# BartvLaatum/GreenLight-Gym2

Measured on AMD Instinct MI355X. Metric: TomatoEnv env-steps/sec, higher is better.
Workload: dtype f32

## Files before the change

### greenlight-gym2_amd/csrc/glgym.hip

```cpp
#include <hip/hip_runtime.h>

#include <cmath>
#include <cstdio>
#include <cstdlib>
#include <cstring>
#include <new>
#include <string>
#include <vector>

#include "glgym.h"
#include "gl_model.hpp"
#include "gl_model_quad.hpp"
#include "gl_reward.hpp"
#include "glgym_bdf.h"
#include "glgym_rng.h"
#include "glgym_plan.h"

using namespace glm;

namespace {

thread_local std::string g_err;

#define HIPCHK(expr)                                                                                   \
    do {                                                                                               \
        hipError_t e_ = (expr);                                                                        \
        if (e_ != hipSuccess) {                                                                        \
            g_err = std::string(#expr) + ": " + hipGetErrorString(e_);                                 \
            return GLGYM_EHIP;                                                                         \
        }                                                                                              \
    } while (0)

constexpr int WAVE = 64;

#include "gl_default_const.inc"
static_assert(sizeof(ModelConst<float>) == sizeof(kDefaultConstF32_image), "regenerate gl_default_const.inc");
static_assert(sizeof(ModelConst<double>) == sizeof(kDefaultConstF64_image), "regenerate gl_default_const.inc");
template <class T> struct DefaultConst;
template <> struct DefaultConst<float> {
    static constexpr ModelConst<float> value = __builtin_bit_cast(ModelConst<float>, kDefaultConstF32_bits);
};
template <> struct DefaultConst<double> {
    static constexpr ModelConst<double> value = __builtin_bit_cast(ModelConst<double>, kDefaultConstF64_bits);
};
__constant__ const ModelConst<float> g_default_f32 = __builtin_bit_cast(ModelConst<float>, kDefaultConstF32_bits);
__constant__ const ModelConst<double> g_default_f64 = __builtin_bit_cast(ModelConst<double>, kDefaultConstF64_bits);
template <class T> __device__ __forceinline__ const ModelConst<T>& device_default();
template <> __device__ __forceinline__ const ModelConst<float>& device_default<float>() { return g_default_f32; }
template <> __device__ __forceinline__ const ModelConst<double>& device_default<double>() { return g_default_f64; }

template <class T> struct RewardConst : RewardConstBase<T> {};

template <class T> struct StepArgsT {
    int B, ld;
    T* x; T* u;
// ... 482 lines not shown
    T k[NX];
    rhs<T, true, PIPE>(x0, s, m, cr, k);
    for (int i = 0; i < NX; ++i) dx[(size_t)b * NX + i] = (double)k[i];
}

template <class T, bool PER_ENV_CROP, bool PIPE = false, int SCH = 0>
__global__ __launch_bounds__(WAVE) void evalf_kernel(const double* x, const double* u, const double* d,
                                                     const double* crop, int B, T dt, int n_sub, T gasR, T tCanMin,
                                                     ModelConst<T> m, double* x_next, int rhs_only, int nd,
                                                     int* n_failed, int verify, int window)
{
    const int b = blockIdx.x * WAVE + threadIdx.x;
    if (b >= B) return;
    T x0[NX], uu[NU], dd[7];
    for (int i = 0; i < NX; ++i) x0[i] = T(x[(size_t)b * NX + i]);
    for (int i = 0; i < NU; ++i) uu[i] = T(u[(size_t)b * NU + i]);
    for (int i = 0; i < 7; ++i) dd[i] = T(d[(size_t)b * nd + i]);
    CropConst<T> crLocal;
    if (PER_ENV_CROP) {
        T pc[NCROP];
        for (int i = 0; i < NCROP; ++i) pc[i] = T(crop[(size_t)b * NCROP + i]);
        make_crop_const<T, T>(pc, gasR, tCanMin, crLocal);
    }
    const CropConst<T>& cr = PER_ENV_CROP ? crLocal : m.crop;
    StepCoef<T> s;
    precompute(uu, dd, m, cr, s);
    if (PIPE) {
        const T tPipe = T(d[(size_t)b * nd + 10]), swOff = T(d[(size_t)b * nd + 12]);
        s.pipeTrack = ((tPipe < T(1)) || (swOff > T(0))) ? T(0) : T(1);
        s.tPipeSet = tPipe;
    }
    if (rhs_only) {
        T k[NX];
        rhs<T, true, PIPE>(x0, s, m, cr, k);
        for (int i = 0; i < NX; ++i) x_next[(size_t)b * NX + i] = (double)k[i];
        return;
    }
    T del[NX];
    bool failed;
    rk4_delta_guarded<T, PIPE, gl_order(SCH), SchemeWin<T, SCH>::value>(x0, s, m, cr, dt, n_sub, del, &failed, nullptr, verify != 0, nullptr, window);
    for (int i = 0; i < NX; ++i)
        x_next[(size_t)b * NX + i] = failed ? __builtin_nan("") : (double)x0[i] + (double)del[i];
    if (failed) atomicAdd(n_failed, 1);
}

template <class T> struct ObsArgsT {
    int B, ld;
    const T* x; const T* u; const T* weather; int weather_rows;
    const int* w_off; const int* timestep; const float* start_day;
    int Np; float* obs; double doy_inc, hod_inc;
    const unsigned char* mask; float* term_obs;
    int nd;
    int moff[6], dim;
};

#ifndef GL_OBS_ROWS
#define GL_OBS_ROWS 16
#endif
constexpr int OBS_ROWS = GL_OBS_ROWS, OBS_NCORE = 23, OBS_MAX_NP = 128;
template <class T> __global__ __launch_bounds__(256) void obs_kernel(ObsArgsT<T> a)
{
    constexpr int ROWS = OBS_ROWS, NCORE = OBS_NCORE;
    extern __shared__ float4 span4[];
    float* span = reinterpret_cast<float*>(span4);
    const int tid = threadIdx.x;
    const int dim = a.dim;
    const float kPpm = (float)(8.3144598 / (101325.0 * 44.01e-3));
    for (int rb = blockIdx.x * ROWS; rb < a.B; rb += gridDim.x * ROWS) {
        const int nrows = min(ROWS, a.B - rb);
        if (a.mask) {
            int any = 0;
            for (int r = 0; r < nrows; ++r) any |= a.mask[rb + r];
            if (!any) continue;
        }
        int base_r[ROWS];
#pragma unroll
        for (int r = 0; r < ROWS; ++r) {
            const int b = rb + (r < nrows ? r : 0);
            const int ts = a.timestep[b];
            base_r[r] = a.w_off[b] + (ts > 0 ? ts - 1 : 0);
        }
        for (int e = tid; e < ROWS * NCORE; e += 256) {
            const int r = e / NCORE, j = e - r * NCORE;
            const int b = rb + (r < nrows ? r : 0);
            const int ts = a.timestep[b];
            const int k = ts > 0 ? ts - 1 : 0;
            int base = 0;
#pragma unroll
            for (int rr = 0; rr < ROWS; ++rr) base = (rr == r) ? base_r[rr] : base;
            base = base >= a.weather_rows ? a.weather_rows - 1 : (base < 0 ? 0 : base);
            const T* wrow = a.weather + (size_t)base * a.nd;
            const int xi = j == 0 ? 0 : j == 1 ? 2 : j == 2 ? 15 : j == 3 ? 9 : j == 4 ? 21 : j == 5 ? 25 : 26;
            const T* p1 = j < 7 ? a.x + (size_t)xi * a.ld + b
                                : (j < 13 ? a.u + (size_t)(j - 7) * a.ld + b : wrow + (j < 18 ? j - 13 : 0));
            const T* p2 = j < 13 ? a.x + (size_t)2 * a.ld + b : wrow + 1;
            const float prim = (float)*p1, aux = (float)*p2, sday = a.start_day[b];
            const float sat = 610.78f * __builtin_amdgcn_exp2f(1.44269504f * 17.2694f * aux * __builtin_amdgcn_rcpf(aux + 238.3f));
            const float rh = fminf(fmaxf(100.0f * prim * __builtin_amdgcn_rcpf(sat), 0.0f), 100.0f);
            const float ppm = kPpm * (aux + 273.15f) * prim;
            const int c = j - 18;
            const double rev = (c <= 2) ? ((double)sday + (double)ts * a.doy_inc) * (1.0 / 365.0)
                                        : (double)ts * a.hod_inc * (1.0 / 24.0);
            const float fr = (float)(rev - floor(rev));
            const float clk = (c == 1 || c == 3) ? __builtin_amdgcn_sinf(fr) : __builtin_amdgcn_cosf(fr);
            float v = prim;
            v = (j == 0 || j == 16) ? ppm : v;
            v = (j == 2 || j == 15) ? rh : v;
            v = (j == 18) ? (float)k : v;
            v = (j > 18) ? clk : v;
            const int mo = j < 4 ? a.moff[0] : j < 7 ? a.moff[1] : j < 13 ? a.moff[2] : j < 18 ? a.moff[3] : a.moff[4];
            const int jl = j < 4 ? j : j < 7 ? j - 4 : j < 13 ? j - 7 : j < 18 ? j - 13 : j - 18;
            if (r < nrows && mo >= 0) span[r * dim + mo + jl] = v;
        }
        const int nf = a.moff[5] >= 0 ? 5 * a.Np : 0;
        for (int q = tid; q < nf; q += 256) {
            const int i = q / 5, c = q - i * 5;
            float v[ROWS];
#pragma unroll
            for (int r = 0; r < ROWS; ++r) {
                int row = base_r[r] + 1 + i;
                row = row >= a.weather_rows ? a.weather_rows - 1 : (row < 0 ? 0 : row);
                v[r] = (float)a.weather[(size_t)row * a.nd + c];
            }
#pragma unroll
            for (int r = 0; r < ROWS; ++r)
                if (r < nrows) span[r * dim + a.moff[5] + q] = v[r];
        }
        __syncthreads();
        float* out = a.obs + (size_t)rb * dim;
        if (!a.mask && nrows == ROWS) {
            const int n4 = (ROWS * dim) >> 2;
            float4* out4 = reinterpret_cast<float4*>(out);
            typedef float v4f __attribute__((ext_vector_type(4)));
            const v4f* src4 = reinterpret_cast<const v4f*>(span4);
            v4f* dst4 = reinterpret_cast<v4f*>(out4);
            for (int e = tid; e < n4; e += 256) __builtin_nontemporal_store(src4[e], &dst4[e]);
        } else {
            for (int r = 0; r < nrows; ++r) {
                if (a.mask && !a.mask[rb + r]) continue;
                for (int jj = tid; jj < dim; jj += 256) {
                    const size_t e = (size_t)r * dim + jj;
                    if (a.mask && a.term_obs) a.term_obs[(size_t)rb * dim + e] = out[e];
                    out[e] = span[e];
                }
            }
        }
        __syncthreads();
    }
}

template <class T>
__global__ __launch_bounds__(256) void rule_based_kernel(glgym_rule_cfg c, int B, int ld, const T* __restrict__ x,
                                                         const T* __restrict__ weather, int weather_rows,
                                                         const int* __restrict__ w_off, const int* __restrict__ timestep,
                                                         const float* __restrict__ start_day, const double* hour,
                                                         const double* doy_in, double doy_inc, double hod_inc,
                                                         T* __restrict__ control, int nd)
{
    const int b = blockIdx.x * blockDim.x + threadIdx.x;
    if (b >= B) return;
    const int ts = timestep[b];
    int row = w_off[b] + ts;
    row = row >= weather_rows ? weather_rows - 1 : (row < 0 ? 0 : row);
    const T* w = weather + (size_t)row * nd;
    const double iGlob = (double)w[0], tOut = (double)w[1], dli = (double)w[7], isDay = (double)w[8],
                 isDaySmooth = (double)w[9];
    const double co2Air = (double)x[b], tAir = (double)x[(size_t)2 * ld + b], vpAir = (double)x[(size_t)15 * ld + b];
    const double hod = hour ? hour[b] : fmod((double)ts * hod_inc, 24.0);
    const double doy = doy_in ? doy_in[b] : (double)start_day[b] + (double)ts * doy_inc;
    auto pband = [](double v, double sp, double band, double lo, double hi) {
        return lo + (hi - lo) * (1.0 / (1.0 + exp(-2.0 / band * 4.605170185988092 * (v - sp - band * 0.5))));
    };
    const double tod = c.lamps_on <= c.lamps_off ? (double)(c.lamps_on < hod && hod < c.lamps_off)
                                                 : (double)(c.lamps_on < hod || hod < c.lamps_off);
    const double doy_ok = c.lamps_day_start <= c.lamps_day_stop
                              ? (double)(c.lamps_day_start < doy && doy < c.lamps_day_stop)
                              : (double)(c.lamps_day_start < doy || doy < c.lamps_day_stop);
    const double below_dli = (double)(dli < c.lamp_rad_sum_limit);
    const double lamp_no_cons = (double)(iGlob < c.lamps_off_sun) * below_dli * tod * doy_ok;
    const double sw_on = fmax(0.0, fmin(1.0, hod - c.lamps_on + 1.0));
    const double sw_off = fmax(0.0, fmin(1.0, c.lamps_off - hod + 1.0));
    const double both = c.lamps_on == c.lamps_off ? 0.0
                        : (c.lamps_on < c.lamps_off ? fmin(sw_on, sw_off) : fmax(sw_on, sw_off));
    const double smooth_lamp = both * below_dli * doy_ok;
    const double day_inside = fmax(smooth_lamp, isDay);
    const double heat_sp = day_inside * c.temp_setpoint_day + (1.0 - day_inside) * c.temp_setpoint_night +
                           c.heat_correction * lamp_no_cons;
    const double heat_max = heat_sp + c.heat_deadzone;
    const double co2_sp = day_inside * c.co2_day;
    const double co2_ppm = 1e6 * 8.3144598 * (tAir + 273.15) * (1e-6 * co2Air) / (101325.0 * 44.01e-3);
    const double rh_in = 100.0 * vpAir / (610.78 * exp(17.2694 * tAir / (tAir + 238.3)));
    const double vent_heat = pband(tAir, heat_max, c.vent_heat_Pband, 0, 1);
    const double vent_rh = pband(rh_in, c.rh_max + 0.0 * c.mech_dehumid_Pband, c.vent_rh_Pband, 0, 1);
    const double vent_cold = pband(tAir, heat_sp - c.t_vent_off, c.vent_cold_Pband, 1, 0);
    const double th_sp = isDay * c.thScrSpDay + (1.0 - isDay) * c.thScrSpNight;
    const double th_cold = pband(tOut, th_sp, c.thScrPband, 0, 1);
    const double th_heat = pband(tAir, heat_sp + c.thScrDeadZone, -c.thScrPband, 1, 0);
    const double th_rh = fmax(pband(rh_in, c.rhMax + c.thScrRh, c.thScrRhPband, 1, 0), 1.0 - vent_cold);
    const double lamp_on = lamp_no_cons * pband(tAir, heat_max + c.lampExtraHeat, -0.5, 0, 1) *
                           (isDaySmooth + (1.0 - isDaySmooth)) *
// ... 914 lines not shown
        g_err = "glgym_step: GLGYM_INTEGRATOR_BDF does not support GLGYM_ODE_PIPE";
        return GLGYM_EINVAL;
    }
    glbdf::BdfEnvArgs<T> k;
    k.ld = a->ld;
    k.x = (T*)a->x; k.u = (T*)a->u; k.action = a->action; k.control = (const T*)a->control;
    k.weather = (const T*)a->weather; k.weather_rows = a->weather_rows; k.nd = h->nd;
    k.w_off = a->w_off; k.timestep = a->timestep; k.crop_p = (const T*)a->crop_p; k.N = a->N;
    k.reward = (T*)a->reward; k.info = (T*)a->info; k.done = a->done; k.step_flags = a->step_flags;
    k.dt = h->dt; k.rtol = h->rtol; k.atol = h->atol; k.max_steps = h->max_steps;
    k.gasR = h->p[39]; k.tCanMin = h->p[162];
    k.du = h->du;
    for (int j = 0; j < NU; ++j) { k.u_min[j] = h->u_min[j]; k.u_max[j] = h->u_max[j]; }
    HIPCHK(bdf_env_launch<T>(k, a->B, h->md, rw, a->metrics, st));
    return GLGYM_OK;
}

extern "C" int glgym_step(glgym_handle h, const glgym_step_args* a, void* stream)
{
    if (!h || !a) { g_err = "glgym_step: null handle / arguments"; return GLGYM_EINVAL; }
    if (a->struct_size != (int32_t)sizeof(glgym_step_args)) {
        g_err = "glgym_step: glgym_step_args.struct_size is " + std::to_string(a->struct_size) + ", this library expects " +
                std::to_string(sizeof(glgym_step_args)) + " (ABI " + std::to_string(GLGYM_ABI_VERSION) + "): rebuild against include/glgym.h";
        return GLGYM_EINVAL;
    }
    if (a->B < 1 || a->ld < a->B || !a->x || !a->u || !a->weather || !a->w_off || !a->timestep ||
        !a->reward || !a->done || (!a->action) == (!a->control) || a->weather_rows < 1) {
        g_err = "glgym_step: bad arguments (exactly one of action/control, ld >= B, non-null state/outputs)";
        return GLGYM_EINVAL;
    }
    if (h->step_integrator == GLGYM_INTEGRATOR_BDF) {
        DeviceGuard dev_guard(h);
        return h->dtype == GLGYM_F32 ? launch_step_bdf<float>(h, a, h->rf, (hipStream_t)stream)
                                     : launch_step_bdf<double>(h, a, h->rd, (hipStream_t)stream);
    }
    if (h->integrator != GLGYM_INTEGRATOR_EXPLICIT) {
        g_err = "glgym_step: GLGYM_INTEGRATOR_BDF is available to glgym_evalF only; set GLGYM_INTEGRATOR_EXPLICIT for env-steps";
        return GLGYM_EINVAL;
    }
    DeviceGuard dev_guard(h);
    hipStream_t st = (hipStream_t)stream;
    return h->dtype == GLGYM_F32 ? launch_step<float>(h, a, h->mf, h->rf, st)
                                 : launch_step<double>(h, a, h->md, h->rd, st);
}

static const int OBS_MODULE_SIZE[6] = {4, 3, 6, 5, 5, 0};

template <class T> static int launch_obs(glgym_handle h, const glgym_obs_args* a, hipStream_t st)
{
    ObsArgsT<T> k;
    k.B = a->B; k.ld = a->ld; k.x = (const T*)a->x; k.u = (const T*)a->u; k.weather = (const T*)a->weather;
    k.weather_rows = a->weather_rows; k.w_off = a->w_off; k.timestep = a->timestep; k.start_day = a->start_day;
    k.Np = a->Np; k.obs = a->obs; k.mask = a->mask; k.term_obs = a->term_obs; k.doy_inc = std::fmod(h->dt / 86400.0, 365.0); k.hod_inc = h->dt / 3600.0; k.nd = h->nd;
    int blocks = (a->B + OBS_ROWS - 1) / OBS_ROWS;
    static const int cap = [] { const char* e = std::getenv("GLGYM_OBS_BLOCKS"); return e ? std::atoi(e) : 4096; }();
    if (blocks > cap) blocks = cap;
    for (int m = 0; m < 6; ++m) k.moff[m] = -1;
    k.dim = 0;
    for (int i = 0; i < h->n_obs_modules; ++i) {
        const int m = h->obs_modules[i];
        k.moff[m] = k.dim;
        k.dim += m == GLGYM_OBS_FORECAST ? 5 * a->Np : OBS_MODULE_SIZE[m];
    }
    const size_t lds = (size_t)OBS_ROWS * k.dim * sizeof(float);
    hipLaunchKernelGGL((obs_kernel<T>), dim3(blocks), dim3(256), lds, st, k);
    HIPCHK(hipGetLastError());
    return GLGYM_OK;
}



extern "C" int glgym_weather(glgym_handle h, const glgym_weather_args* a, void* stream)
{
    DeviceGuard dev_guard(h);
    if (!h || !a || a->n_raw < 3 || a->n_out < 1 || a->nd < ND || !a->time || !a->i_glob || !a->t_out || !a->rh || !a->wind ||
        !a->t_sky || !a->out || !a->workspace) {
        g_err = "glgym_weather: bad arguments (>= 3 raw samples, nd >= 10, non-null device pointers)";
        return GLGYM_EINVAL;
    }
    hipStream_t st = (hipStream_t)stream;
    const int n = a->n_raw;
    double* W = a->workspace;
    double* D = a->workspace + (size_t)10 * n;
    hipLaunchKernelGGL(weather_convert_kernel, dim3((n + 255) / 256), dim3(256), 0, st, n, a->time, a->i_glob, a->t_out,
                       a->rh, a->wind, a->t_sky, a->co2_ppm, W);
    hipLaunchKernelGGL(weather_scan_kernel, dim3(1), dim3(64), 0, st, n, a->time, W);
    hipLaunchKernelGGL(pchip_slopes_kernel, dim3((n + 255) / 256, 10), dim3(256), 0, st, n, 10, a->time, W, D);
    if (a->nd > ND) {
        HIPCHK(hipMemsetAsync(a->out, 0, (size_t)a->n_out * a->nd * (h->dtype == GLGYM_F32 ? 4 : 8), st));
    }
    const dim3 grid((a->n_out + 255) / 256, 10);
    if (h->dtype == GLGYM_F32)
        hipLaunchKernelGGL((pchip_eval_kernel<float>), grid, dim3(256), 0, st, n, 10, a->n_out, a->nd, a->time, W, D,
                           (float*)a->out);
    else
        hipLaunchKernelGGL((pchip_eval_kernel<double>), grid, dim3(256), 0, st, n, 10, a->n_out, a->nd, a->time, W, D,
                           (double*)a->out);
    HIPCHK(hipGetLastError());
    return GLGYM_OK;
}

extern "C" int glgym_vecnorm(glgym_handle h, const glgym_vecnorm_args* a, void* stream)
{
    DeviceGuard dev_guard(h);
    if (!h || !a || a->B < 1 || a->dim < 1 || !a->obs || !a->obs_out || !a->obs_mean || !a->obs_var || !a->obs_count ||
        !a->workspace || (a->reward && (!a->reward_out || !a->ret_stats || !a->returns))) {
        g_err = "glgym_vecnorm: bad arguments";
        return GLGYM_EINVAL;
    }
    hipStream_t st = (hipStream_t)stream;
    const int B = a->B, dim = a->dim;
    double* acc = a->workspace;
    double* acc2 = a->workspace + (size_t)VN_REP * 2 * dim;
    HIPCHK(hipMemsetAsync(a->workspace, 0, ((size_t)VN_REP * 2 * dim + 2) * sizeof(double), st));
    const int do_obs = a->training && a->norm_obs, do_ret = a->training && a->reward != nullptr;
    int col_threads = (dim + WAVE - 1) / WAVE * WAVE;
    if (col_threads > 1024) col_threads = 1024;
    if (do_obs) {
        int blocks = (B + 63) / 64;
        if (blocks > 1024) blocks = 1024;
        hipLaunchKernelGGL(vecnorm_moments_kernel, dim3(blocks), dim3(col_threads), 0, st, a->obs, B, dim, acc);
    }
    if (do_ret) {
        if (h->dtype == GLGYM_F32)
            hipLaunchKernelGGL((vecnorm_returns_kernel<float>), dim3((B + 255) / 256), dim3(256), 0, st,
                               (const float*)a->reward, a->returns, B, a->gamma, acc2);
        else
            hipLaunchKernelGGL((vecnorm_returns_kernel<double>), dim3((B + 255) / 256), dim3(256), 0, st,
                               (const double*)a->reward, a->returns, B, a->gamma, acc2);
    }
    double* scale = acc;
    if (do_obs || do_ret || a->norm_obs)
        hipLaunchKernelGGL(vecnorm_merge_kernel, dim3(1), dim3(1024), 0, st, a->obs_mean, a->obs_var, a->obs_count, acc, dim, B,
                           a->ret_stats, acc2, do_obs, do_ret, a->epsilon, a->norm_obs ? scale : nullptr);
    const size_t total = (size_t)B * dim;
    if (a->norm_obs) {
        int blocks = (B + 15) / 16;
        if (blocks > 8192) blocks = 8192;
        hipLaunchKernelGGL(vecnorm_apply_kernel, dim3(blocks), dim3(col_threads), 0, st, a->obs, a->obs_out, B, dim,
                           a->obs_mean, scale, a->clip_obs);
    } else if (a->obs_out != a->obs) {
        HIPCHK(hipMemcpyAsync(a->obs_out, a->obs, total * sizeof(float), hipMemcpyDeviceToDevice, st));
    }
    if (a->reward) {
        if (h->dtype == GLGYM_F32)
            hipLaunchKernelGGL((vecnorm_reward_kernel<float>), dim3((B + 255) / 256), dim3(256), 0, st,
                               (const float*)a->reward, a->reward_out, a->returns, a->done, B, a->ret_stats, a->epsilon,
                               a->clip_reward, a->norm_reward);
        else
            hipLaunchKernelGGL((vecnorm_reward_kernel<double>), dim3((B + 255) / 256), dim3(256), 0, st,
                               (const double*)a->reward, a->reward_out, a->returns, a->done, B, a->ret_stats, a->epsilon,
                               a->clip_reward, a->norm_reward);
    }
    HIPCHK(hipGetLastError());
    return GLGYM_OK;
}

extern "C" {

int glgym_obs(glgym_handle h, const glgym_obs_args* a, void* stream)
{
    DeviceGuard dev_guard(h);
    if (!h || !a || a->B < 1 || a->ld < a->B || !a->x || !a->u || !a->weather || !a->w_off || !a->timestep ||
        !a->start_day || !a->obs || a->Np < 0 || a->Np > OBS_MAX_NP) {
        g_err = "glgym_obs: bad arguments (null pointer, ld < B, or Np outside 0..128)";
        return GLGYM_EINVAL;
    }
    hipStream_t st = (hipStream_t)stream;
    return h->dtype == GLGYM_F32 ? launch_obs<float>(h, a, st) : launch_obs<double>(h, a, st);
}

int glgym_set_obs_modules(glgym_handle h, const int32_t* modules, int n)
{
    if (!h || !modules || n < 1 || n > 6) { g_err = "glgym_set_obs_modules: 1..6 module ids expected"; return GLGYM_EINVAL; }
    int seen = 0;
    for (int i = 0; i < n; ++i) {
        if (modules[i] < 0 || modules[i] > 5 || (seen >> modules[i] & 1)) {
            g_err = "glgym_set_obs_modules: ids must be distinct GLGYM_OBS_* values";
            return GLGYM_EINVAL;
        }
        seen |= 1 << modules[i];
    }
    for (int i = 0; i < n; ++i) h->obs_modules[i] = modules[i];
    h->n_obs_modules = n;
    return GLGYM_OK;
}

int glgym_obs_dim(glgym_handle h, int Np)
{
    if (!h || Np < 0 || Np > OBS_MAX_NP) return GLGYM_EINVAL;
    int dim = 0;
    for (int i = 0; i < h->n_obs_modules; ++i)
        dim += h->obs_modules[i] == GLGYM_OBS_FORECAST ? 5 * Np : OBS_MODULE_SIZE[h->obs_modules[i]];
    return dim;
}

int glgym_reset(glgym_handle h, const glgym_reset_args* a, void* stream)
{
    DeviceGuard dev_guard(h);
    if (!h || !a || a->B < 1 || a->ld < a->B || !a->x || !a->u || !a->timestep || !a->weather || !a->w_off) {
        g_err = "glgym_reset: bad arguments";
        return GLGYM_EINVAL;
    }
    hipStream_t st = (hipStream_t)stream;
    const dim3 grid((a->B + 255) / 256), block(256);
    if (h->dtype == GLGYM_F32)
        hipLaunchKernelGGL((reset_kernel<float>), grid, block, 0, st, a->B, a->ld, a->mask, (float*)a->x, (float*)a->u,
                           a->timestep, (const float*)a->weather, a->weather_rows, a->w_off, a->start_rows, a->start_days,
                           a->n_starts, a->start_day, a->episode, (unsigned long long)a->seed, h->nd);
    else
        hipLaunchKernelGGL((reset_kernel<double>), grid, block, 0, st, a->B, a->ld, a->mask, (double*)a->x,
                           (double*)a->u, a->timestep, (const double*)a->weather, a->weather_rows, a->w_off,
                           a->start_rows, a->start_days, a->n_starts, a->start_day, a->episode,
                           (unsigned long long)a->seed, h->nd);
    HIPCHK(hipGetLastError());
    return GLGYM_OK;
}

// ... 175 lines not shown
```

### greenlight-gym2_amd/csrc/gl_model.hpp

```cpp
#pragma once
#include <cmath>

#if defined(__HIPCC__)
#define GL_HD __host__ __device__ __forceinline__
#else
#define GL_HD inline
#endif

#if defined(__HIP_DEVICE_COMPILE__)
#define GL_WAVE_ANY(c) (__any(c) != 0)
#else
#define GL_WAVE_ANY(c) (c)
#endif


namespace glm {

constexpr int NX = 28, NU = 6, ND = 10, NP = 208;
constexpr int NCROP = 34;
constexpr int CROP0 = 128;

template <class T> struct Math;
template <class T> GL_HD T ceil_pos(T v) { return T(::ceil(v)); }

// ... 1281 lines not shown
    static_assert(ORDER == 5 || ORDER == 4 || ORDER == 3 || ORDER == 2, "ORDER: 5 (five-stage fourth-order 2N scheme), 4 (RK4), 3 (three-stage third-order scheme) or 2 (midpoint rule), all with the cover conduction exponential");
    using M = Math<T>;
    constexpr bool COVEXP = true;
    const int WINR = win_rt > 0 ? win_rt : WIN;
    const T S = ScScheme<T, ORDER>::S(), est_fac = ScScheme<T, ORDER>::est_fac();
    const ScGrid<T> grid = sc_grid<T>(dt, n_sub, WINR);
    const T hw_nom = grid.hw_nom, hnom_nom = grid.hnom_nom;
    T hw = hw_nom, hnom = hnom_nom;
    T t_now = T(0), t_harv = T(0.5) * hw_nom;
    int n_left = 0;
    T y[NX], xs[NX], k[NX], acc[NX], est[SC_NFAST];
    T winc[NX];
    T z0_reg[WBUF ? 1 : NX];
    T* z0 = WBUF ? wbuf : z0_reg;
    if (!WBUF) {
#pragma unroll
        for (int i = 0; i < NX; ++i) z0[i] = x0[i];
        z0[5] = x0[3] - x0[5]; z0[7] = x0[2] - x0[7]; z0[20] = x0[2] - x0[20];
        if (COVEXP) z0[6] = x0[5] - x0[6];
    }
    const T gamCov = m.iCapCov * m.cCovCond;
    T dprev_reg[WBUF ? 1 : GL_N_SLOW], dwin_reg[WBUF ? 1 : GL_N_SLOW];
    T* dprev = WBUF ? wbuf + NX : dprev_reg;
    T* dwin = WBUF ? dprev : dwin_reg;
#pragma unroll
    for (int j = 0; j < GL_N_SLOW; ++j) dprev[j] = T(0);
    SlowCoef<T> q;
#pragma unroll
    for (int i = 0; i < NX; ++i) del[i] = T(0);
#pragma unroll
    for (int j = 0; j < SC_NFAST; ++j) est[j] = T(0);
    int n_steps = 0, flags = 0;
    T t_cap = T(0);
    T h_last = hnom;
    EtdCoef<T> ec;
    LsCoef<T> lc;
    T ls_Nprev = T(0), ls_hprev = T(0);
    T h_ec = T(-1);
    auto state_now = [&]() {
#pragma unroll
        for (int p = 0; p < GL_NPAIR; ++p)
            RkVec<T>::pair(gl_pair_a(p), gl_pair_b(p), [&](auto r) { r.st(y, r.ld(z0) + r.ld(del)); });
    };
    int side_prev = 0;
    bool capped_prev = false;
    del[23] += harvest_flow(z0[23] + del[23], cr.cLeafMax, T(0.5) * hw_nom);
    del[25] += harvest_flow(z0[25] + del[25], cr.cFruitMax, T(0.5) * hw_nom);
    for (int it = 0;; ++it) {
        const T t_left = dt - t_now;
        const bool closing = it > 0 && n_left <= 1;
        flags |= (t_cap > T(SC_CAP_S)) ? SC_FLAG_CAP : 0;
        if (flags & SC_FLAG_CAP) break;
        state_now();
#pragma unroll
        for (int i = 0; i < NX; ++i)
            if (gl_slow_slot(i) >= 0) { xs[i] = y[i] + T(0.5) * dprev[gl_slow_slot(i)]; dwin[gl_slow_slot(i)] = del[i]; }
        slow_coef<T>(xs, s, m, cr, q);
        T lam = hnom_nom;
        int side = capped_prev ? 1 : 0;
        rhs_stage<T, PIPE, true, COVEXP>(y, q, s, m, cr, k, &lam, &side);
        flags |= sc_branch_flag(side_prev, side, capped_prev);
        side_prev = side;
        if (it > 0) {
            T worst = T(0);
#pragma unroll
            for (int j = 0; j < SC_NFAST; ++j) {
                const T wj = ((ORDER == 4 || ORDER == 3) && sc_fast(j) == 6) ? T(sc_itol(j)) * ec.w3 : T(sc_itol(j));
                worst = M::max(worst, M::abs(est[j] - k[sc_fast(j)]) * wj);
            }
            flags |= sc_estimate_flag<T>(grid, worst, h_last, est_fac, t_now);
        }
        if (closing) break;
        sc_window_length<T>(grid, S, lam, t_left, it == 0, hw, hnom, n_left);
        auto fast_move = [&](const T* kk, T w_at) {
            T mv = T(0);
#pragma unroll
            for (int j = 0; j < SC_NFAST; ++j)
                if (j != 7) {
                    T kj = kk[sc_fast(j)];
                    if (COVEXP && sc_fast(j) == 5) kj = kk[5] - T(0.5) * kk[6] + gamCov * w_at;
                    if (COVEXP && sc_fast(j) == 6) kj = (kk[3] - kk[5]) - T(0.5) * kk[6] + gamCov * w_at;
                    mv = M::max(mv, M::abs(kj) * T(sc_itol(j)));
                }
            return mv;
        };
        const ScPlan<T> plan = sc_plan<T, ORDER>(grid, S, lam, hw, hnom, fast_move(k, y[6]));
        const bool capped = plan.capped;
        t_cap += capped ? hw : T(0);
        capped_prev = capped;
        T n_rem = plan.n_rem;
        T h = plan.h;
        h_last = h;
        const bool adaptive = plan.adaptive;
        T t_rem = hw;
        T w_now = y[6];
        if (ORDER == 5) {
#pragma unroll
            for (int p = 0; p < GL_NPAIR_FAST; ++p) RkVec<T>::pair(gl_pair_a(p), gl_pair_b(p), [&](auto r) { r.st(winc, r.sp(T(0))); });
        }
        if (COVEXP && h != h_ec) {
            if (ORDER == 5) ls_coefs<T>(T(2) * gamCov, h, lc); else etd_coefs<T>(T(2) * gamCov, h, ec);
            h_ec = h;
        }
        auto sub_step = [&]() {
            const T h2 = T(0.5) * h;
            if (ORDER == 5) {
                const T w0 = w_now, N0 = k[6];
                const T F0 = N0 - (T(2) * gamCov) * w0;
                const T slope = (h <= T(2.0001) * ls_hprev) ? (N0 - ls_Nprev) * M::rcp(ls_hprev) : T(0);
// ... 111 lines not shown
                for (int j = 0; j < SC_NFAST; ++j) est[j] = -k[sc_fast(j)];
                const T w0 = y[6];
#pragma unroll
                for (int p = 0; p < GL_NPAIR_FAST; ++p)
                    if (p != 3)
                        RkVec<T>::pair(gl_pair_a(p), gl_pair_b(p), [&](auto r) { r.st(xs, r.ld(y) + r.sp(h2) * r.ld(k)); });
                {
                    const T dWa = ec.e2m1 * w0 + ec.q * k[6];
                    xs[5] = y[5] + h2 * k[5] - T(0.5) * dWa; xs[6] = w0 + dWa;
                }
                rhs_stage<T, PIPE, false, COVEXP>(xs, q, s, m, cr, k);
#pragma unroll
                for (int p = 0; p < GL_NPAIR; ++p)
                    if (p != 3)
                        RkVec<T>::pair(gl_pair_a(p), gl_pair_b(p), [&](auto r) { r.st(del, r.ld(del) + r.sp(h) * r.ld(k)); });
                {
                    const T dW = ec.em1 * w0 + ec.hp1 * k[6];
                    del[6] += dW;
                    del[5] += h * k[5] - T(0.5) * dW;
                }
            }
            ++n_steps;
        };
        sub_step();
        t_rem -= h;
#pragma unroll
        for (int j = 0; j < SC_NFAST; ++j) est[j] = (ORDER != 2) ? k[sc_fast(j)] : est[j] + T(2.0) * k[sc_fast(j)];
        for (n_rem -= T(1); n_rem >= T(0.5); n_rem -= T(1)) {
            if (ORDER == 5) {
#pragma unroll
                for (int p = 0; p < GL_NPAIR_FAST; ++p)
                    RkVec<T>::pair(gl_pair_a(p), gl_pair_b(p), [&](auto r) { r.st(xs, r.ld(y) + r.ld(winc)); });
                w_now = xs[6];
                rhs_stage<T, PIPE, false, COVEXP>(xs, q, s, m, cr, k);
            } else {
                state_now();
                rhs_stage<T, PIPE, false, COVEXP>(y, q, s, m, cr, k);
            }
            if (ORDER == 5 && GL_WAVE_ANY(adaptive)) {
                sc_replan<T>(grid, plan, adaptive, t_rem, fast_move(k, w_now), h, n_rem);
                h_last = h;
                if (h != h_ec) { ls_coefs<T>(T(2) * gamCov, h, lc); h_ec = h; }
            }
            sub_step();
            t_rem -= h;
#pragma unroll
            for (int j = 0; j < SC_NFAST; ++j) est[j] = (ORDER != 2) ? k[sc_fast(j)] : est[j] + T(2.0) * k[sc_fast(j)];
        }
        if (ORDER == 5) {
#pragma unroll
            for (int p = 0; p < GL_NPAIR_FAST; ++p)
                RkVec<T>::pair(gl_pair_a(p), gl_pair_b(p), [&](auto r) { r.st(del, r.ld(del) + r.ld(winc)); });
        }
#pragma unroll
        for (int i = 0; i < NX; ++i)
            if (gl_slow_slot(i) >= 0) dprev[gl_slow_slot(i)] = del[i] - dwin[gl_slow_slot(i)];
        t_now = (n_left <= 1) ? dt : t_now + hw;
        const T hh = sc_harvest_advance<T>(dt, t_now, hw, t_harv);
        del[23] += harvest_flow(z0[23] + del[23], cr.cLeafMax, hh);
        del[25] += harvest_flow(z0[25] + del[25], cr.cFruitMax, hh);
    }
    del[5] = del[3] - del[5]; del[7] = del[2] - del[7]; del[20] = del[2] - del[20];
    if (COVEXP) del[6] = del[5] - del[6];
    del[NX - 1] = dt * T(1.0 / 86400.0);
    st.n_steps = n_steps;
    st.flags = flags;
}

template <class T> GL_HD bool all_finite(const T* v)
{
    T chk = T(0);
#pragma unroll
    for (int i = 0; i < NX; ++i) chk += v[i] * T(0);
    return chk == T(0);
}

template <class T, bool PIPE = false, int ORDER = 4, int WIN = 1, bool WBUF = false>
GL_HD int rk4_delta_guarded(const T* x0, const StepCoef<T>& s, const ModelConst<T>& m, const CropConst<T>& cr, T dt,
                            int n_sub, T* del, bool* failed, int* extra_steps = nullptr, bool verify = false,
                            int* first_flags = nullptr, int win_rt = 0, T* wbuf = nullptr)
{
    using M = Math<T>;
    const int WINR = win_rt > 0 ? win_rt : WIN;
    ScLadder L = sc_ladder_start(n_sub);
    T prev[SC_NFAST];
#pragma unroll
    for (int j = 0; j < SC_NFAST; ++j) prev[j] = T(0);
    for (int attempt = 0; attempt < SC_ATTEMPTS; ++attempt) {
        if (L.done) break;
        ScStat<T> st;
        rk_delta<T, PIPE, ORDER, WIN, WBUF>(x0, s, m, cr, dt, L.n, del, st, win_rt, wbuf);
        T worst = T(0);
#pragma unroll
        for (int j = 0; j < SC_NFAST; ++j) worst = M::max(worst, M::abs(del[sc_fast(j)] - prev[j]) * T(sc_itol(j)));
        sc_ladder_judge<T>(L, attempt, st.flags, st.n_steps, WINR, all_finite(del), worst, verify, first_flags);
#pragma unroll
        for (int j = 0; j < SC_NFAST; ++j) prev[j] = del[sc_fast(j)];
    }
    *failed = !L.ok;
    if (extra_steps) *extra_steps = sc_ladder_extra_steps(L, n_sub, WINR);
    return L.extra;
}

template <class T, bool PIPE = false>
GL_HD void rk4_delta(const T* x0, const StepCoef<T>& s, const ModelConst<T>& m, const CropConst<T>& cr, T dt,
                     int n_sub, T* del)
{
    ScStat<T> st;
    rk_delta<T, PIPE, 4, 1>(x0, s, m, cr, dt, n_sub, del, st);
// ... 4 lines not shown
```

Measured before the change: 101.1 million.

## Restructure observation kernel to per-wavefront strips with ballot-based masked dispatch

The observation kernel now assigns each 4-row strip to a single wavefront. It uses wave-level barriers in place of block-wide __syncthreads, and prefetches the core inputs into registers while overlapping them with the forecast gather. In masked mode, teams of waves use ballot to pick strips that have active rows, so fully masked rows are skipped cheaply. Separate masked and unmasked template instantiations and a lower default block count are meant to cut sync overhead and idle threads, at the cost of more registers per thread and more complex code.

```diff
diff --git a/greenlight-gym2_amd/csrc/glgym.hip b/greenlight-gym2_amd/csrc/glgym.hip
--- a/greenlight-gym2_amd/csrc/glgym.hip
+++ b/greenlight-gym2_amd/csrc/glgym.hip
@@ -1,6 +1,8 @@
 #include <hip/hip_runtime.h>
 
+#include <algorithm>
 #include <cmath>
+#include <cstdint>
 #include <cstdio>
 #include <cstdlib>
 #include <cstring>
@@ -589,100 +591,173 @@
     const unsigned char* mask; float* term_obs;
     int nd;
     int moff[6], dim;
+    int vec16, mask4;
 };
 
-#ifndef GL_OBS_ROWS
-#define GL_OBS_ROWS 16
+#ifndef GL_OBS_TEAM
+#define GL_OBS_TEAM 8
 #endif
-constexpr int OBS_ROWS = GL_OBS_ROWS, OBS_NCORE = 23, OBS_MAX_NP = 128;
-template <class T> __global__ __launch_bounds__(256) void obs_kernel(ObsArgsT<T> a)
+constexpr int OBS_BLOCKS_DEFAULT = 2048;
+constexpr int OBS_ROWS = 4, OBS_NCORE = 23, OBS_MAX_NP = 128, OBS_TEAM = GL_OBS_TEAM;
+static_assert(OBS_TEAM >= 4 && OBS_TEAM <= 64 && (OBS_TEAM & (OBS_TEAM - 1)) == 0, "OBS_TEAM: a power of two, one block (4 wavefronts) at least");
+
+__device__ __forceinline__ void obs_wave_sync()
+{
+    __builtin_amdgcn_fence(__ATOMIC_RELEASE, "wavefront");
+    __builtin_amdgcn_wave_barrier();
+    __builtin_amdgcn_fence(__ATOMIC_ACQUIRE, "wavefront");
+}
+
+template <class T, bool MASKED>
+__device__ __forceinline__ void obs_strip(const ObsArgsT<T>& a, float4* span4, int rb, int nrows, unsigned flags, int lane)
 {
     constexpr int ROWS = OBS_ROWS, NCORE = OBS_NCORE;
-    extern __shared__ float4 span4[];
     float* span = reinterpret_cast<float*>(span4);
-    const int tid = threadIdx.x;
     const int dim = a.dim;
     const float kPpm = (float)(8.3144598 / (101325.0 * 44.01e-3));
-    for (int rb = blockIdx.x * ROWS; rb < a.B; rb += gridDim.x * ROWS) {
-        const int nrows = min(ROWS, a.B - rb);
-        if (a.mask) {
-            int any = 0;
-            for (int r = 0; r < nrows; ++r) any |= a.mask[rb + r];
-            if (!any) continue;
-        }
-        int base_r[ROWS];
-#pragma unroll
-        for (int r = 0; r < ROWS; ++r) {
-            const int b = rb + (r < nrows ? r : 0);
-            const int ts = a.timestep[b];
-            base_r[r] = a.w_off[b] + (ts > 0 ? ts - 1 : 0);
-        }
-        for (int e = tid; e < ROWS * NCORE; e += 256) {
-            const int r = e / NCORE, j = e - r * NCORE;
-            const int b = rb + (r < nrows ? r : 0);
-            const int ts = a.timestep[b];
-            const int k = ts > 0 ? ts - 1 : 0;
-            int base = 0;
-#pragma unroll
-            for (int rr = 0; rr < ROWS; ++rr) base = (rr == r) ? base_r[rr] : base;
-            base = base >= a.weather_rows ? a.weather_rows - 1 : (base < 0 ? 0 : base);
-            const T* wrow = a.weather + (size_t)base * a.nd;
-            const int xi = j == 0 ? 0 : j == 1 ? 2 : j == 2 ? 15 : j == 3 ? 9 : j == 4 ? 21 : j == 5 ? 25 : 26;
-            const T* p1 = j < 7 ? a.x + (size_t)xi * a.ld + b
-                                : (j < 13 ? a.u + (size_t)(j - 7) * a.ld + b : wrow + (j < 18 ? j - 13 : 0));
-            const T* p2 = j < 13 ? a.x + (size_t)2 * a.ld + b : wrow + 1;
-            const float prim = (float)*p1, aux = (float)*p2, sday = a.start_day[b];
-            const float sat = 610.78f * __builtin_amdgcn_exp2f(1.44269504f * 17.2694f * aux * __builtin_amdgcn_rcpf(aux + 238.3f));
-            const float rh = fminf(fmaxf(100.0f * prim * __builtin_amdgcn_rcpf(sat), 0.0f), 100.0f);
-            const float ppm = kPpm * (aux + 273.15f) * prim;
-            const int c = j - 18;
-            const double rev = (c <= 2) ? ((double)sday + (double)ts * a.doy_inc) * (1.0 / 365.0)
-                                        : (double)ts * a.hod_inc * (1.0 / 24.0);
-            const float fr = (float)(rev - floor(rev));
-            const float clk = (c == 1 || c == 3) ? __builtin_amdgcn_sinf(fr) : __builtin_amdgcn_cosf(fr);
-            float v = prim;
-            v = (j == 0 || j == 16) ? ppm : v;
-            v = (j == 2 || j == 15) ? rh : v;
-            v = (j == 18) ? (float)k : v;
-            v = (j > 18) ? clk : v;
-            const int mo = j < 4 ? a.moff[0] : j < 7 ? a.moff[1] : j < 13 ? a.moff[2] : j < 18 ? a.moff[3] : a.moff[4];
-            const int jl = j < 4 ? j : j < 7 ? j - 4 : j < 13 ? j - 7 : j < 18 ? j - 13 : j - 18;
-            if (r < nrows && mo >= 0) span[r * dim + mo + jl] = v;
-        }
-        const int nf = a.moff[5] >= 0 ? 5 * a.Np : 0;
-        for (int q = tid; q < nf; q += 256) {
+    int ts_r[ROWS], base_r[ROWS];
+#pragma unroll
+    for (int r = 0; r < ROWS; ++r) {
+        const int b = rb + (r < nrows ? r : 0);
+        ts_r[r] = a.timestep[b];
+        base_r[r] = a.w_off[b] + (ts_r[r] > 0 ? ts_r[r] - 1 : 0);
+    }
+    constexpr int NC = (ROWS * NCORE + WAVE - 1) / WAVE;
+    int c_r[NC], c_j[NC], c_ts[NC];
+    float c_prim[NC], c_aux[NC], c_sday[NC];
+#pragma unroll
+    for (int h = 0; h < NC; ++h) {
+        const int e = lane + h * WAVE < ROWS * NCORE ? lane + h * WAVE : 0;
+        const int r = e / NCORE, j = e - r * NCORE;
+        const int b = rb + (r < nrows ? r : 0);
+        int ts = 0, base = 0;
+#pragma unroll
+        for (int rr = 0; rr < ROWS; ++rr) { ts = (rr == r) ? ts_r[rr] : ts; base = (rr == r) ? base_r[rr] : base; }
+        base = base >= a.weather_rows ? a.weather_rows - 1 : (base < 0 ? 0 : base);
+        const T* wrow = a.weather + (size_t)base * a.nd;
+        const int xi = j == 0 ? 0 : j == 1 ? 2 : j == 2 ? 15 : j == 3 ? 9 : j == 4 ? 21 : j == 5 ? 25 : 26;
+        const T* s1 = j < 7 ? a.x + (size_t)xi * a.ld + b : a.u + (size_t)(j < 13 ? j - 7 : 0) * a.ld + b;
+        const T* w1 = wrow + (j >= 13 && j < 18 ? j - 13 : 0);
+        const T sv1 = *s1, sv2 = a.x[(size_t)2 * a.ld + b], wv1 = *w1, wv2 = wrow[1];
+        c_prim[h] = (float)(j < 13 ? sv1 : wv1); c_aux[h] = (float)(j < 13 ? sv2 : wv2);
+        c_sday[h] = a.start_day[b];
+        c_r[h] = r; c_j[h] = j; c_ts[h] = ts;
+    }
+    const int nf = a.moff[5] >= 0 ? 5 * a.Np : 0;
+    auto gather = [&](int q0, float (&v)[2][ROWS]) {
+#pragma unroll
+        for (int h = 0; h < 2; ++h) {
+            const int q = q0 + h * WAVE < nf ? q0 + h * WAVE : 0;
             const int i = q / 5, c = q - i * 5;
-            float v[ROWS];
 #pragma unroll
             for (int r = 0; r < ROWS; ++r) {
                 int row = base_r[r] + 1 + i;
                 row = row >= a.weather_rows ? a.weather_rows - 1 : (row < 0 ? 0 : row);
-                v[r] = (float)a.weather[(size_t)row * a.nd + c];
+                v[h][r] = (float)a.weather[(size_t)row * a.nd + c];
             }
+        }
+    };
+    auto scatter = [&](int q0, const float (&v)[2][ROWS]) {
+#pragma unroll
+        for (int h = 0; h < 2; ++h) {
+            const int q = q0 + h * WAVE;
 #pragma unroll
             for (int r = 0; r < ROWS; ++r)
-                if (r < nrows) span[r * dim + a.moff[5] + q] = v[r];
-        }
-        __syncthreads();
-        float* out = a.obs + (size_t)rb * dim;
-        if (!a.mask && nrows == ROWS) {
-            const int n4 = (ROWS * dim) >> 2;
-            float4* out4 = reinterpret_cast<float4*>(out);
-            typedef float v4f __attribute__((ext_vector_type(4)));
-            const v4f* src4 = reinterpret_cast<const v4f*>(span4);
-            v4f* dst4 = reinterpret_cast<v4f*>(out4);
-            for (int e = tid; e < n4; e += 256) __builtin_nontemporal_store(src4[e], &dst4[e]);
-        } else {
-            for (int r = 0; r < nrows; ++r) {
-                if (a.mask && !a.mask[rb + r]) continue;
-                for (int jj = tid; jj < dim; jj += 256) {
-                    const size_t e = (size_t)r * dim + jj;
-                    if (a.mask && a.term_obs) a.term_obs[(size_t)rb * dim + e] = out[e];
-                    out[e] = span[e];
-                }
+                if (q < nf && r < nrows) span[r * dim + a.moff[5] + q] = v[h][r];
+        }
+    };
+    float fv[2][ROWS];
+    gather(lane, fv);
+#pragma unroll
+    for (int h = 0; h < NC; ++h) {
+        const int r = c_r[h], j = c_j[h], ts = c_ts[h];
+        const int k = ts > 0 ? ts - 1 : 0;
+        const float prim = c_prim[h], aux = c_aux[h], sday = c_sday[h];
+        const float sat = 610.78f * __builtin_amdgcn_exp2f(1.44269504f * 17.2694f * aux * __builtin_amdgcn_rcpf(aux + 238.3f));
+        const float rh = fminf(fmaxf(100.0f * prim * __builtin_amdgcn_rcpf(sat), 0.0f), 100.0f);
+        const float ppm = kPpm * (aux + 273.15f) * prim;
+        const int c = j - 18;
+        const double rev = (c <= 2) ? ((double)sday + (double)ts * a.doy_inc) * (1.0 / 365.0)
+                                    : (double)ts * a.hod_inc * (1.0 / 24.0);
+        const float fr = (float)(rev - floor(rev));
+        const float clk = (c == 1 || c == 3) ? __builtin_amdgcn_sinf(fr) : __builtin_amdgcn_cosf(fr);
+        float v = prim;
+        v = (j == 0 || j == 16) ? ppm : v;
+        v = (j == 2 || j == 15) ? rh : v;
+        v = (j == 18) ? (float)k : v;
+        v = (j > 18) ? clk : v;
+        const int mo = j < 4 ? a.moff[0] : j < 7 ? a.moff[1] : j < 13 ? a.moff[2] : j < 18 ? a.moff[3] : a.moff[4];
+        const int jl = j < 4 ? j : j < 7 ? j - 4 : j < 13 ? j - 7 : j < 18 ? j - 13 : j - 18;
+        if (lane + h * WAVE < ROWS * NCORE && r < nrows && mo >= 0) span[r * dim + mo + jl] = v;
+    }
+    scatter(lane, fv);
+    for (int q0 = lane + 2 * WAVE; q0 < nf; q0 += 2 * WAVE) {
+        gather(q0, fv);
+        scatter(q0, fv);
+    }
+    obs_wave_sync();
+    float* out = a.obs + (size_t)rb * dim;
+    float* term = MASKED && a.term_obs ? a.term_obs + (size_t)rb * dim : nullptr;
+    const bool all_rows = nrows == ROWS && (!MASKED || ((flags & 0xffu) && (flags & 0xff00u) && (flags & 0xff0000u) && (flags >> 24)));
+    if (all_rows && a.vec16) {
+        typedef float v4f __attribute__((ext_vector_type(4)));
+        const v4f* src4 = reinterpret_cast<const v4f*>(span4);
+        v4f* dst4 = reinterpret_cast<v4f*>(out);
+        v4f* term4 = reinterpret_cast<v4f*>(term);
+        for (int e = lane; e < dim; e += WAVE) {
+            if (MASKED) {
+                if (term) term4[e] = dst4[e];
+                dst4[e] = src4[e];
+            } else {
+                __builtin_nontemporal_store(src4[e], &dst4[e]);
             }
         }
-        __syncthreads();
+    } else {
+        for (int r = 0; r < nrows; ++r) {
+            if (MASKED && !((flags >> (8 * r)) & 0xffu)) continue;
+            for (int jj = lane; jj < dim; jj += WAVE) {
+                const int e = r * dim + jj;
+                if (term) term[e] = out[e];
+                out[e] = span[e];
+            }
+        }
+    }
+    obs_wave_sync();
+}
+
+template <class T, bool MASKED> __global__ __launch_bounds__(256) void obs_kernel(ObsArgsT<T> a)
+{
+    extern __shared__ float4 span_all[];
+    const int lane = threadIdx.x & (WAVE - 1);
+    const int wv = __builtin_amdgcn_readfirstlane(threadIdx.x >> 6);
+    float4* span4 = span_all + wv * a.dim;
+    const int gw = blockIdx.x * 4 + wv, nw = gridDim.x * 4;
+    const int nstrips = (a.B + OBS_ROWS - 1) / OBS_ROWS;
+    if (!MASKED) {
+        for (int s = gw; s < nstrips; s += nw)
+            obs_strip<T, false>(a, span4, s * OBS_ROWS, min(OBS_ROWS, a.B - s * OBS_ROWS), 0x01010101u, lane);
+    } else {
+        const int nseg = (nstrips + WAVE - 1) / WAVE;
+        unsigned long long share = 0;
+        for (int i = gw % OBS_TEAM; i < WAVE; i += OBS_TEAM) share |= 1ull << i;
+        for (int seg = gw / OBS_TEAM; seg < nseg; seg += nw / OBS_TEAM) {
+            const int b = (seg * WAVE + lane) * OBS_ROWS;
+            unsigned mw = 0;
+            if (a.mask4 && b + OBS_ROWS <= a.B) {
+                mw = *reinterpret_cast<const unsigned*>(a.mask + b);
+            } else {
+                for (int r = 0; r < OBS_ROWS; ++r)
+                    if (b + r < a.B && a.mask[b + r]) mw |= 1u << (8 * r);
+            }
+            unsigned long long work = __builtin_amdgcn_ballot_w64(mw != 0) & share;
+            while (work) {
+                const int l = __builtin_ctzll(work);
+                work &= work - 1;
+                const unsigned flags = __builtin_amdgcn_readlane(mw, l);
+                const int rb = (seg * WAVE + l) * OBS_ROWS;
+                obs_strip<T, true>(a, span4, rb, min(OBS_ROWS, a.B - rb), flags, lane);
+            }
+        }
     }
 }
 
@@ -1703,9 +1778,17 @@
     k.B = a->B; k.ld = a->ld; k.x = (const T*)a->x; k.u = (const T*)a->u; k.weather = (const T*)a->weather;
     k.weather_rows = a->weather_rows; k.w_off = a->w_off; k.timestep = a->timestep; k.start_day = a->start_day;
     k.Np = a->Np; k.obs = a->obs; k.mask = a->mask; k.term_obs = a->term_obs; k.doy_inc = std::fmod(h->dt / 86400.0, 365.0); k.hod_inc = h->dt / 3600.0; k.nd = h->nd;
-    int blocks = (a->B + OBS_ROWS - 1) / OBS_ROWS;
-    static const int cap = [] { const char* e = std::getenv("GLGYM_OBS_BLOCKS"); return e ? std::atoi(e) : 4096; }();
-    if (blocks > cap) blocks = cap;
+    const int nstrips = (a->B + OBS_ROWS - 1) / OBS_ROWS;
+    static const int cap = [] { const char* e = std::getenv("GLGYM_OBS_BLOCKS"); const int v = e ? std::atoi(e) : 0; return v > 0 ? v : OBS_BLOCKS_DEFAULT; }();
+    int blocks;
+    if (!a->mask) {
+        blocks = std::min((nstrips + 3) / 4, cap);
+    } else {
+        blocks = (nstrips + WAVE - 1) / WAVE * (OBS_TEAM / 4);
+        blocks = std::min(blocks, std::max(cap / (OBS_TEAM / 4), 1) * (OBS_TEAM / 4));
+    }
+    k.vec16 = (((uintptr_t)a->obs | (uintptr_t)(a->mask ? a->term_obs : nullptr)) & 15) == 0;
+    k.mask4 = ((uintptr_t)a->mask & 3) == 0;
     for (int m = 0; m < 6; ++m) k.moff[m] = -1;
     k.dim = 0;
     for (int i = 0; i < h->n_obs_modules; ++i) {
@@ -1713,8 +1796,11 @@
         k.moff[m] = k.dim;
         k.dim += m == GLGYM_OBS_FORECAST ? 5 * a->Np : OBS_MODULE_SIZE[m];
     }
-    const size_t lds = (size_t)OBS_ROWS * k.dim * sizeof(float);
-    hipLaunchKernelGGL((obs_kernel<T>), dim3(blocks), dim3(256), lds, st, k);
+    const size_t lds = (size_t)4 * OBS_ROWS * k.dim * sizeof(float);
+    if (a->mask)
+        hipLaunchKernelGGL((obs_kernel<T, true>), dim3(blocks), dim3(256), lds, st, k);
+    else
+        hipLaunchKernelGGL((obs_kernel<T, false>), dim3(blocks), dim3(256), lds, st, k);
     HIPCHK(hipGetLastError());
     return GLGYM_OK;
 }
```

After: 102.0 million, median of 6. Within noise of the previous version (+0.8%).

## Restructure obs kernel to map thread groups per row and batch forecast loads

Applied to the files above, without the earlier changes.

Rewrites the observation kernel so each row is handled by a fixed group of threads. Each thread loads its row's timestep, offsets and state values once, instead of every thread recomputing a per-row base index through an unrolled select over all rows. Forecast gathering now runs per row, with many independent loads in flight per thread and 32-bit byte offsets. Masked-block skipping uses a wave ballot, and out-of-range stores go to a spare LDS dummy slot, which needs 16 extra bytes. The change also adds a compile-time-off ablation switch in the model (a timing-only build with wrong results) and a guard rejecting weather tables over 4 GiB.

```diff
diff --git a/greenlight-gym2_amd/csrc/gl_model.hpp b/greenlight-gym2_amd/csrc/gl_model.hpp
--- a/greenlight-gym2_amd/csrc/gl_model.hpp
+++ b/greenlight-gym2_amd/csrc/gl_model.hpp
@@ -1357,9 +1357,16 @@
         flags |= (t_cap > T(SC_CAP_S)) ? SC_FLAG_CAP : 0;
         if (flags & SC_FLAG_CAP) break;
         state_now();
+#ifndef GL_ABLATE_WINBOOK
 #pragma unroll
         for (int i = 0; i < NX; ++i)
             if (gl_slow_slot(i) >= 0) { xs[i] = y[i] + T(0.5) * dprev[gl_slow_slot(i)]; dwin[gl_slow_slot(i)] = del[i]; }
+#else
+#warning "GL_ABLATE_WINBOOK: timing-only build of rk_delta, its results are wrong -- never ship this library"
+#pragma unroll
+        for (int i = 0; i < NX; ++i)
+            if (gl_slow_slot(i) >= 0) xs[i] = y[i];
+#endif
         slow_coef<T>(xs, s, m, cr, q);
         T lam = hnom_nom;
         int side = capped_prev ? 1 : 0;
@@ -1577,9 +1584,11 @@
             for (int p = 0; p < GL_NPAIR_FAST; ++p)
                 RkVec<T>::pair(gl_pair_a(p), gl_pair_b(p), [&](auto r) { r.st(del, r.ld(del) + r.ld(winc)); });
         }
+#ifndef GL_ABLATE_WINBOOK
 #pragma unroll
         for (int i = 0; i < NX; ++i)
             if (gl_slow_slot(i) >= 0) dprev[gl_slow_slot(i)] = del[i] - dwin[gl_slow_slot(i)];
+#endif
         t_now = (n_left <= 1) ? dt : t_now + hw;
         const T hh = sc_harvest_advance<T>(dt, t_now, hw, t_harv);
         del[23] += harvest_flow(z0[23] + del[23], cr.cLeafMax, hh);
diff --git a/greenlight-gym2_amd/csrc/glgym.hip b/greenlight-gym2_amd/csrc/glgym.hip
--- a/greenlight-gym2_amd/csrc/glgym.hip
+++ b/greenlight-gym2_amd/csrc/glgym.hip
@@ -598,40 +598,75 @@
 template <class T> __global__ __launch_bounds__(256) void obs_kernel(ObsArgsT<T> a)
 {
     constexpr int ROWS = OBS_ROWS, NCORE = OBS_NCORE;
+    constexpr int TPR = 256 / ROWS;
+    constexpr int NE = (NCORE + TPR - 1) / TPR;
+    constexpr int NG = 15;
+    static_assert(ROWS >= 8 && ROWS <= 64 && (ROWS & (ROWS - 1)) == 0, "OBS_ROWS: a power of two, a multiple of 8, at most one wave");
     extern __shared__ float4 span4[];
     float* span = reinterpret_cast<float*>(span4);
     const int tid = threadIdx.x;
+    const int r = tid / TPR, l = tid - r * TPR;
     const int dim = a.dim;
     const float kPpm = (float)(8.3144598 / (101325.0 * 44.01e-3));
     for (int rb = blockIdx.x * ROWS; rb < a.B; rb += gridDim.x * ROWS) {
         const int nrows = min(ROWS, a.B - rb);
         if (a.mask) {
-            int any = 0;
-            for (int r = 0; r < nrows; ++r) any |= a.mask[rb + r];
-            if (!any) continue;
-        }
-        int base_r[ROWS];
-#pragma unroll
-        for (int r = 0; r < ROWS; ++r) {
-            const int b = rb + (r < nrows ? r : 0);
-            const int ts = a.timestep[b];
-            base_r[r] = a.w_off[b] + (ts > 0 ? ts - 1 : 0);
-        }
-        for (int e = tid; e < ROWS * NCORE; e += 256) {
-            const int r = e / NCORE, j = e - r * NCORE;
-            const int b = rb + (r < nrows ? r : 0);
-            const int ts = a.timestep[b];
-            const int k = ts > 0 ? ts - 1 : 0;
-            int base = 0;
-#pragma unroll
-            for (int rr = 0; rr < ROWS; ++rr) base = (rr == r) ? base_r[rr] : base;
-            base = base >= a.weather_rows ? a.weather_rows - 1 : (base < 0 ? 0 : base);
-            const T* wrow = a.weather + (size_t)base * a.nd;
+            const int rr = tid & (ROWS - 1);
+            const int mk = a.mask[rb + (rr < nrows ? rr : 0)];
+            if (__ballot(mk != 0) == 0) continue;
+        }
+        const bool row_ok = r < nrows;
+        const int b = rb + (row_ok ? r : 0);
+        const int ts = a.timestep[b];
+        const int w_off = a.w_off[b];
+        const float sday = a.start_day[b];
+        const float t_air = (float)a.x[(size_t)2 * a.ld + b];
+        float p_xu[NE];
+#pragma unroll
+        for (int n = 0; n < NE; ++n) {
+            const int j = min(l + n * TPR, NCORE - 1);
             const int xi = j == 0 ? 0 : j == 1 ? 2 : j == 2 ? 15 : j == 3 ? 9 : j == 4 ? 21 : j == 5 ? 25 : 26;
-            const T* p1 = j < 7 ? a.x + (size_t)xi * a.ld + b
-                                : (j < 13 ? a.u + (size_t)(j - 7) * a.ld + b : wrow + (j < 18 ? j - 13 : 0));
-            const T* p2 = j < 13 ? a.x + (size_t)2 * a.ld + b : wrow + 1;
-            const float prim = (float)*p1, aux = (float)*p2, sday = a.start_day[b];
+            const T* p = j < 7 ? a.x + (size_t)xi * a.ld + b : (j < 13 ? a.u + (size_t)(j - 7) * a.ld + b : a.x + b);
+            p_xu[n] = (float)*p;
+        }
+        const int k = ts > 0 ? ts - 1 : 0;
+        const int base_r = w_off + k;
+        const int base = base_r >= a.weather_rows ? a.weather_rows - 1 : (base_r < 0 ? 0 : base_r);
+        const T* wrow = a.weather + (size_t)base * a.nd;
+        const float t_out = (float)wrow[1];
+        float p_w[NE];
+#pragma unroll
+        for (int n = 0; n < NE; ++n) {
+            const int j = min(l + n * TPR, NCORE - 1);
+            p_w[n] = (float)wrow[(j >= 13 && j < 18) ? j - 13 : 0];
+        }
+        const int nf = a.moff[5] >= 0 ? 5 * a.Np : 0;
+        const int n_chunk = (nf + TPR * NG - 1) / (TPR * NG);
+        const char* wbytes = reinterpret_cast<const char*>(a.weather);
+        const int nf_l = row_ok ? nf : 0;
+        float* frow = span + r * dim + a.moff[5];
+        for (int ch = 0; ch < n_chunk; ++ch) {
+            const int q0 = l + ch * (TPR * NG);
+            float v[NG];
+#pragma unroll
+            for (int g = 0; g < NG; ++g) {
+                const int q = min(q0 + g * TPR, nf - 1);
+                const int i = q / 5, c = q - i * 5;
+                int row = base_r + 1 + i;
+                row = row >= a.weather_rows ? a.weather_rows - 1 : (row < 0 ? 0 : row);
+                const unsigned off = ((unsigned)row * (unsigned)a.nd + (unsigned)c) * (unsigned)sizeof(T);
+                v[g] = (float)*reinterpret_cast<const T*>(wbytes + off);
+            }
+#pragma unroll
+            for (int g = 0; g < NG; ++g) {
+                const int q = q0 + g * TPR;
+                *(q < nf_l ? frow + q : span + ROWS * dim) = v[g];
+            }
+        }
+#pragma unroll
+        for (int n = 0; n < NE; ++n) {
+            const int j = l + n * TPR;
+            const float prim = j < 13 ? p_xu[n] : p_w[n], aux = j < 13 ? t_air : t_out;
             const float sat = 610.78f * __builtin_amdgcn_exp2f(1.44269504f * 17.2694f * aux * __builtin_amdgcn_rcpf(aux + 238.3f));
             const float rh = fminf(fmaxf(100.0f * prim * __builtin_amdgcn_rcpf(sat), 0.0f), 100.0f);
             const float ppm = kPpm * (aux + 273.15f) * prim;
@@ -647,21 +682,7 @@
             v = (j > 18) ? clk : v;
             const int mo = j < 4 ? a.moff[0] : j < 7 ? a.moff[1] : j < 13 ? a.moff[2] : j < 18 ? a.moff[3] : a.moff[4];
             const int jl = j < 4 ? j : j < 7 ? j - 4 : j < 13 ? j - 7 : j < 18 ? j - 13 : j - 18;
-            if (r < nrows && mo >= 0) span[r * dim + mo + jl] = v;
-        }
-        const int nf = a.moff[5] >= 0 ? 5 * a.Np : 0;
-        for (int q = tid; q < nf; q += 256) {
-            const int i = q / 5, c = q - i * 5;
-            float v[ROWS];
-#pragma unroll
-            for (int r = 0; r < ROWS; ++r) {
-                int row = base_r[r] + 1 + i;
-                row = row >= a.weather_rows ? a.weather_rows - 1 : (row < 0 ? 0 : row);
-                v[r] = (float)a.weather[(size_t)row * a.nd + c];
-            }
-#pragma unroll
-            for (int r = 0; r < ROWS; ++r)
-                if (r < nrows) span[r * dim + a.moff[5] + q] = v[r];
+            span[(row_ok && j < NCORE && mo >= 0) ? r * dim + mo + jl : ROWS * dim] = v;
         }
         __syncthreads();
         float* out = a.obs + (size_t)rb * dim;
@@ -1713,7 +1734,7 @@
         k.moff[m] = k.dim;
         k.dim += m == GLGYM_OBS_FORECAST ? 5 * a->Np : OBS_MODULE_SIZE[m];
     }
-    const size_t lds = (size_t)OBS_ROWS * k.dim * sizeof(float);
+    const size_t lds = (size_t)OBS_ROWS * k.dim * sizeof(float) + 16;
     hipLaunchKernelGGL((obs_kernel<T>), dim3(blocks), dim3(256), lds, st, k);
     HIPCHK(hipGetLastError());
     return GLGYM_OK;
@@ -1815,6 +1836,10 @@
     if (!h || !a || a->B < 1 || a->ld < a->B || !a->x || !a->u || !a->weather || !a->w_off || !a->timestep ||
         !a->start_day || !a->obs || a->Np < 0 || a->Np > OBS_MAX_NP) {
         g_err = "glgym_obs: bad arguments (null pointer, ld < B, or Np outside 0..128)";
+        return GLGYM_EINVAL;
+    }
+    if ((unsigned long long)a->weather_rows * h->nd * (h->dtype == GLGYM_F32 ? 4 : 8) > 0xffffffffULL) {
+        g_err = "glgym_obs: weather table of more than 4 GiB";
         return GLGYM_EINVAL;
     }
     hipStream_t st = (hipStream_t)stream;
```

After: 100.5 million before, 101.7 million after, median of 6. About the same (+1.2%).
